# neuronika/neuronika

Hardware: NVIDIA H100
Metric: forward+backward GFLOP/s (higher is better)
Workload: dtype bf16

## Files before the change

neuronika_b200/csrc/nk_gemm_tc.cu:

```cuda
#include "nk_internal.cuh"
#include "nk_ptx.cuh"

namespace {

constexpr int BLOCK_M = 128;
constexpr int BLOCK_K = 64;
constexpr int WGMMA_K = 16;
constexpr int kNumThreads = 384;
constexpr uint32_t kSmemLimit = 232448;
constexpr int kEpiCols = 64;
constexpr uint32_t kEpiStageBytes = 2 * 64 * kEpiCols * 4;

struct GemmParams {
  int64_t M, N, K;
  int64_t ldc;
  void* C;
  const void* bias;
  float alpha, beta;
  int bias_bf16;
  int bias_per_row;
  int relu;
  const void* mask;
  float* colsum;
  int num_m_blocks, num_n_blocks, num_k_blocks;
  uint32_t a_lbo, a_sbo, a_kstep;
  uint32_t b_lbo, b_sbo, b_kstep;
  int rs_world, m_rot;
  int64_t rs_rows;
  void* rs_dst[8];
  int batch, a_batched, b_batched, batch_reduce, splits;
  int64_t c_batch_stride;
  int tma_store;
};

__device__ __forceinline__ int tile_m_block(const GemmParams& p, int tile) {
  const int t = tile % p.num_m_blocks;
  if (p.rs_world == 0) return t;
  const int owner = (t + p.m_rot) % p.rs_world;
  return owner * (p.num_m_blocks / p.rs_world) + t / p.rs_world;
}

constexpr int kGroupM = 16;
__device__ __forceinline__ void tile_coords(const GemmParams& p, int tile, int& m_blk, int& n_blk) {
  if (p.rs_world) {
    m_blk = tile_m_block(p, tile);
    n_blk = tile / p.num_m_blocks;
    return;
  }
  const int group_size = kGroupM * p.num_n_blocks;
  const int group = tile / group_size, in_group = tile - group * group_size;
  const int first_m = group * kGroupM;
  const int gm = min(p.num_m_blocks - first_m, kGroupM);
  m_blk = first_m + in_group % gm;
  n_blk = in_group / gm;
}

template <int BLOCK_N>
struct Cfg {
  static constexpr uint32_t A_BYTES = BLOCK_M * BLOCK_K * 2;
  static constexpr uint32_t B_BYTES = BLOCK_N * BLOCK_K * 2;
  static constexpr uint32_t STAGE_BYTES = A_BYTES + B_BYTES;
  static constexpr int kStagesMax = (kSmemLimit - 2048 - kEpiStageBytes) / STAGE_BYTES;
  static constexpr int kStages = kStagesMax > 8 ? 8 : kStagesMax;
  static constexpr uint32_t SMEM_BYTES = kStages * STAGE_BYTES + 2048 + kEpiStageBytes;
};

__device__ __forceinline__ void scale_and_bias(const GemmParams& p, int64_t row, int64_t col0, const uint32_t* r, bool full,
                                               float* v) {
#pragma unroll
  for (int j = 0; j < 32; ++j) v[j] = __fmul_rn(p.alpha, __uint_as_float(r[j]));
  if (p.bias && p.bias_per_row) {
    const float b = p.bias_bf16 ? __bfloat162float(static_cast<const __nv_bfloat16*>(p.bias)[row]) : static_cast<const float*>(p.bias)[row];
#pragma unroll
    for (int j = 0; j < 32; ++j) v[j] += b;
  } else if (p.bias) {
    if (full && (reinterpret_cast<uintptr_t>(p.bias) & 15) == 0) {
      if (p.bias_bf16) {
        const uint4* bp = reinterpret_cast<const uint4*>(static_cast<const __nv_bfloat16*>(p.bias) + col0);
#pragma unroll
        for (int q = 0; q < 4; ++q) {
          const uint4 w = __ldg(bp + q);
          const uint32_t ww[4] = {w.x, w.y, w.z, w.w};
#pragma unroll
          for (int i = 0; i < 4; ++i) {
            v[q * 8 + 2 * i] += __uint_as_float(ww[i] << 16);
            v[q * 8 + 2 * i + 1] += __uint_as_float(ww[i] & 0xffff0000u);
          }
        }
      } else {
        const float4* bp = reinterpret_cast<const float4*>(static_cast<const float*>(p.bias) + col0);
#pragma unroll
        for (int q = 0; q < 8; ++q) {
          const float4 w = __ldg(bp + q);
          v[q * 4] += w.x, v[q * 4 + 1] += w.y, v[q * 4 + 2] += w.z, v[q * 4 + 3] += w.w;
        }
      }
    } else {
#pragma unroll
      for (int j = 0; j < 32; ++j)
        if (col0 + j < p.N)
          v[j] += p.bias_bf16 ? __bfloat162float(static_cast<const __nv_bfloat16*>(p.bias)[col0 + j])
                              : static_cast<const float*>(p.bias)[col0 + j];
    }
  }
}

template <typename TC>
__device__ __forceinline__ void epilogue_colsum_chunk32(const GemmParams& p, int64_t row, int64_t col0, const uint32_t* r,
                                                        int lane, bool vec_ok) {
  float v[32];
  const bool live = row < p.M;
  const TC* mrow = (p.mask && live) ? static_cast<const TC*>(p.mask) + row * p.ldc + col0 : nullptr;
  const bool full = col0 + 32 <= p.N;
#pragma unroll
  for (int j = 0; j < 32; ++j) v[j] = (live && col0 + j < p.N) ? p.alpha * __uint_as_float(r[j]) : 0.f;
  if (mrow) {
    if (full && vec_ok) {
      constexpr int V = 16 / sizeof(TC);
#pragma unroll
      for (int q = 0; q < 32 / V; ++q) {
        NkVec<TC> mk;
        mk.load(mrow + q * V);
#pragma unroll
        for (int i = 0; i < V; ++i) v[q * V + i] = mk.get(i) > 0.f ? v[q * V + i] : 0.f;
      }
    } else {
#pragma unroll
      for (int j = 0; j < 32; ++j)
        if (col0 + j < p.N) v[j] = nk_to_f32<TC>(mrow[j]) > 0.f ? v[j] : 0.f;
    }
  }
#pragma unroll
  for (int j = 0; j < 32; ++j) v[j] = nk_to_f32<TC>(nk_from_f32<TC>(v[j]));
#pragma unroll
  for (int off = 16; off >= 1; off >>= 1) {
    const bool upper = (lane & off) != 0;
#pragma unroll
    for (int i = 0; i < off; ++i) {
      const float send = upper ? v[i] : v[i + off];
      const float keep = upper ? v[i + off] : v[i];
      v[i] = keep + __shfl_xor_sync(0xffffffffu, send, off);
    }
  }
  if (col0 + lane < p.N) atomicAdd(p.colsum + col0 + lane, v[0]);
}

template <typename TC>
__device__ __forceinline__ void epilogue_store_chunk32(const GemmParams& p, int64_t row, int64_t col0, const uint32_t* r,
                                                       int ncols, bool vec_ok, int64_t c_off = 0, bool atomic = false) {
  TC* crow = static_cast<TC*>(p.C) + c_off + row * p.ldc + col0;
  if (atomic) {
    if constexpr (sizeof(TC) == 4) {
#pragma unroll
      for (int j = 0; j < 32; ++j)
        if (j < ncols && col0 + j < p.N) atomicAdd(reinterpret_cast<float*>(crow) + j, p.alpha * __uint_as_float(r[j]));
    }
    return;
  }
  if (p.rs_world) {
    const int owner = int(row / p.rs_rows);
    crow = static_cast<TC*>(p.rs_dst[owner]) + (row - owner * p.rs_rows) * p.ldc + col0;
  }
  float v[32];
  const bool full = (col0 + 32 <= p.N) && ncols == 32;
  scale_and_bias(p, row, col0, r, full, v);
  const TC* mrow = p.mask ? static_cast<const TC*>(p.mask) + row * p.ldc + col0 : nullptr;
  if (full && vec_ok) {
    constexpr int V = 16 / sizeof(TC);
    if (mrow) {
#pragma unroll
      for (int q = 0; q < 32 / V; ++q) {
        NkVec<TC> mk;
        mk.load(mrow + q * V);
#pragma unroll
        for (int i = 0; i < V; ++i) v[q * V + i] = mk.get(i) > 0.f ? v[q * V + i] : 0.f;
      }
    }
    if (p.beta != 0.f) {
#pragma unroll
      for (int q = 0; q < 32 / V; ++q) {
        NkVec<TC> c;
        c.load(crow + q * V);
#pragma unroll
        for (int i = 0; i < V; ++i) v[q * V + i] += p.beta * c.get(i);
      }
    }
    if (p.relu) {
#pragma unroll
      for (int j = 0; j < 32; ++j) v[j] = v[j] > 0.f ? v[j] : 0.f;
    }
#pragma unroll
    for (int q = 0; q < 32 / V; ++q) {
      NkVec<TC> o;
#pragma unroll
      for (int i = 0; i < V; ++i) o.set(i, v[q * V + i]);
      o.store(crow + q * V);
    }
  } else {
#pragma unroll
    for (int j = 0; j < 32; ++j) {
      if (j < ncols && col0 + j < p.N) {
        float x = v[j];
        if (mrow) x = nk_to_f32<TC>(mrow[j]) > 0.f ? x : 0.f;
        if (p.beta != 0.f) x += p.beta * nk_to_f32<TC>(crow[j]);
        if (p.relu) x = x > 0.f ? x : 0.f;
        crow[j] = nk_from_f32<TC>(x);
      }
    }
  }
}

__device__ __forceinline__ int epi_index(int row, int col) {
  return row * kEpiCols + ((((col >> 2) ^ (row & 7))) << 2) + (col & 3);
}

__device__ __forceinline__ float col_bias(const GemmParams& p, int64_t col) {
  if (col >= p.N) return 0.f;
  return p.bias_bf16 ? __bfloat162float(static_cast<const __nv_bfloat16*>(p.bias)[col]) : static_cast<const float*>(p.bias)[col];
}

__device__ __forceinline__ float epi_value(const GemmParams& p, float acc, float bias) {
  float v = __fmul_rn(p.alpha, acc);
  if (p.bias) v += bias;
  return p.relu ? (v > 0.f ? v : 0.f) : v;
}

template <int BLOCK_N, bool A_MN, bool B_MN, typename TC, bool BATCH = false>
__global__ void __launch_bounds__(kNumThreads, 1)
gemm_tc_kernel(const __grid_constant__ CUtensorMap tmap_a, const __grid_constant__ CUtensorMap tmap_b,
               const __grid_constant__ CUtensorMap tmap_c, const GemmParams p) {
  using C_ = Cfg<BLOCK_N>;
  constexpr int kStages = C_::kStages;
  constexpr int kStoreCols = 128 / int(sizeof(TC));
  constexpr bool kTmaStore = !BATCH && BLOCK_N % kStoreCols == 0;
  static_assert(2 * 2 * 64 * 128 <= kEpiStageBytes, "staging buffers");
  extern __shared__ uint8_t smem_raw[];
  const uint32_t smem_base = (ptx::smem_u32(smem_raw) + 1023u) & ~1023u;
  const uint32_t smem_a0 = smem_base;
  const uint32_t smem_b0 = smem_base + kStages * C_::A_BYTES;
  const uint32_t bar_base = smem_base + kStages * C_::STAGE_BYTES;
  auto full_bar = [&](int s) { return bar_base + 8u * s; };
  auto empty_bar = [&](int s) { return bar_base + 8u * (kStages + s); };
  const uint32_t epi_stage = bar_base + 1024;
  float* epi = reinterpret_cast<float*>(smem_raw + (epi_stage - ptx::smem_u32(smem_raw)));

  const int wg = threadIdx.x >> 7;
  const int lane = threadIdx.x & 31;

  if (threadIdx.x == 0) {
    ptx::prefetch_tmap(&tmap_a);
    ptx::prefetch_tmap(&tmap_b);
    if (kTmaStore && p.tma_store) ptx::prefetch_tmap(&tmap_c);
    for (int s = 0; s < kStages; ++s) {
      ptx::mbar_init(full_bar(s), 1);
      ptx::mbar_init(empty_bar(s), 2);
    }
    ptx::fence_barrier_init();
  }
  __syncthreads();

  const int tiles_mn = p.num_m_blocks * p.num_n_blocks;
  const int num_tiles = BATCH ? tiles_mn * (p.batch_reduce ? p.splits : p.batch) : tiles_mn;
  auto batch_range = [&](int outer, int& b0, int& b1) {
    if (!p.batch_reduce) {
      b0 = outer, b1 = outer + 1;
    } else {
      const int per = (p.batch + p.splits - 1) / p.splits;
      b0 = outer * per;
      b1 = min(p.batch, b0 + per);
    }
  };

  if (wg == 0) {
    ptx::setmaxnreg_dec<40>();
    if (threadIdx.x == 0) {
      int stage = 0;
      uint32_t phase = 0;
      for (int tile = blockIdx.x; tile < num_tiles; tile += gridDim.x) {
        int m_blk, n_blk, b0 = 0, b1 = 1;
        tile_coords(p, BATCH ? tile % tiles_mn : tile, m_blk, n_blk);
        if (BATCH) batch_range(tile / tiles_mn, b0, b1);
        const int m0 = m_blk * BLOCK_M, n0 = n_blk * BLOCK_N;
        for (int bb = b0; bb < b1; ++bb)
        for (int kb = 0; kb < p.num_k_blocks; ++kb) {
          ptx::mbar_wait_spin(empty_bar(stage), phase ^ 1u);
          ptx::mbar_expect_tx(full_bar(stage), C_::STAGE_BYTES);
          const int k0 = kb * BLOCK_K;
          const uint32_t sa = smem_a0 + stage * C_::A_BYTES;
          const uint32_t sb = smem_b0 + stage * C_::B_BYTES;
          if (A_MN) {
#pragma unroll
            for (int c = 0; c < BLOCK_M / 64; ++c) {
              if (BATCH && p.a_batched)
                ptx::tma_load_3d(sa + c * (64 * BLOCK_K * 2), &tmap_a, full_bar(stage), m0 + c * 64, k0, bb);
              else
                ptx::tma_load_2d(sa + c * (64 * BLOCK_K * 2), &tmap_a, full_bar(stage), m0 + c * 64, k0);
            }
          } else {
            if (BATCH && p.a_batched)
              ptx::tma_load_3d(sa, &tmap_a, full_bar(stage), k0, m0, bb);
            else
              ptx::tma_load_2d(sa, &tmap_a, full_bar(stage), k0, m0);
          }
          if (B_MN) {
#pragma unroll
            for (int c = 0; c < BLOCK_N / 64; ++c) {
              if (BATCH && p.b_batched)
                ptx::tma_load_3d(sb + c * (64 * BLOCK_K * 2), &tmap_b, full_bar(stage), n0 + c * 64, k0, bb);
              else
                ptx::tma_load_2d(sb + c * (64 * BLOCK_K * 2), &tmap_b, full_bar(stage), n0 + c * 64, k0);
            }
          } else {
            if (BATCH && p.b_batched)
              ptx::tma_load_3d(sb, &tmap_b, full_bar(stage), k0, n0, bb);
            else
              ptx::tma_load_2d(sb, &tmap_b, full_bar(stage), k0, n0);
          }
          if (++stage == kStages) {
            stage = 0;
            phase ^= 1u;
          }
        }
      }
    }
    return;
  }

  ptx::setmaxnreg_inc<232>();
  const int cw = wg - 1;
  const int t = threadIdx.x & 127;
  const int warp = t >> 5;
  const bool vec_ok = ((p.ldc * int64_t(sizeof(TC))) % 16 == 0) && ((reinterpret_cast<uintptr_t>(p.C) & 15) == 0) &&
                      ((reinterpret_cast<uintptr_t>(p.mask) & 15) == 0);
  float* stg = epi + cw * (64 * kEpiCols);
  const uint32_t a_off = uint32_t(cw) * (64 * BLOCK_K * 2);
  float acc[BLOCK_N / 2];
  int stage = 0;
  uint32_t phase = 0;
  uint32_t store_buf = 0;
  for (int tile = blockIdx.x; tile < num_tiles; tile += gridDim.x) {
    int m_blk, n_blk;
    tile_coords(p, BATCH ? tile % tiles_mn : tile, m_blk, n_blk);
    int k_total = p.num_k_blocks;
    if (BATCH) {
      int b0, b1;
      batch_range(tile / tiles_mn, b0, b1);
      k_total *= (b1 - b0);
    }
    int prev_stage = 0;
    for (int kb = 0; kb < k_total; ++kb) {
      ptx::mbar_wait_spin(full_bar(stage), phase);
      const uint64_t adesc = ptx::make_smem_desc_sw128(smem_a0 + stage * C_::A_BYTES + a_off, p.a_lbo, p.a_sbo);
      const uint64_t bdesc = ptx::make_smem_desc_sw128(smem_b0 + stage * C_::B_BYTES, p.b_lbo, p.b_sbo);
      ptx::fence_regs(acc);
      ptx::wgmma_fence();
#pragma unroll
      for (int k = 0; k < BLOCK_K / WGMMA_K; ++k)
        ptx::Wgmma<BLOCK_N>::template mma<int(A_MN), int(B_MN)>(acc, adesc + uint64_t((k * p.a_kstep) >> 4),
                                                                 bdesc + uint64_t((k * p.b_kstep) >> 4), (kb | k) != 0 ? 1u : 0u);
      ptx::wgmma_commit();
      ptx::wgmma_wait<1>();
      ptx::fence_regs(acc);
      if (kb > 0 && t == 0) ptx::mbar_arrive(empty_bar(prev_stage));
      prev_stage = stage;
      if (++stage == kStages) {
        stage = 0;
        phase ^= 1u;
      }
    }
    ptx::wgmma_wait<0>();
    ptx::fence_regs(acc);
    if (t == 0) ptx::mbar_arrive(empty_bar(prev_stage));

    if constexpr (kTmaStore) {
      if (p.tma_store) {
        const int fr = warp * 16 + (lane >> 2);
        const int q = lane & 3;
        const int row0 = m_blk * BLOCK_M + cw * 64;
        const uint32_t stg0 = epi_stage + uint32_t(cw) * (2 * 64 * 128);
#pragma unroll
        for (int ch = 0; ch < BLOCK_N / kStoreCols; ++ch) {
          const uint32_t buf = stg0 + store_buf * (64 * 128);
          if (t == 0) ptx::tma_store_wait_read<1>();
          ptx::named_barrier(1 + cw, 128);
          const int64_t col0 = int64_t(n_blk) * BLOCK_N + ch * kStoreCols;
#pragma unroll
          for (int jj = 0; jj < kStoreCols / 8; ++jj) {
            const int j = (ch * (kStoreCols / 8) + jj) * 4;
            const int64_t col = col0 + jj * 8 + 2 * q;
            float b0 = 0.f, b1 = 0.f;
            if (p.bias) b0 = col_bias(p, col), b1 = col_bias(p, col + 1);
            const float v0 = epi_value(p, acc[j], b0), v1 = epi_value(p, acc[j + 1], b1);
            const float v2 = epi_value(p, acc[j + 2], b0), v3 = epi_value(p, acc[j + 3], b1);
            if constexpr (sizeof(TC) == 2) {
              const uint32_t off = fr * 128 + ((jj ^ (fr & 7)) << 4) + 4 * q;
              const __nv_bfloat162 lo = __floats2bfloat162_rn(v0, v1), hi = __floats2bfloat162_rn(v2, v3);
              ptx::st_shared_b32(buf + off, *reinterpret_cast<const uint32_t*>(&lo));
              ptx::st_shared_b32(buf + off + 8 * 128, *reinterpret_cast<const uint32_t*>(&hi));
            } else {
              const uint32_t off = fr * 128 + (((2 * jj + (q >> 1)) ^ (fr & 7)) << 4) + (q & 1) * 8;
              ptx::st_shared_v2_f32(buf + off, v0, v1);
              ptx::st_shared_v2_f32(buf + off + 8 * 128, v2, v3);
            }
          }
          ptx::fence_proxy_async();
          ptx::named_barrier(1 + cw, 128);
          if (t == 0) {
            if (row0 < p.M && col0 < p.N) ptx::tma_store_2d(&tmap_c, buf, int(col0), row0);
            ptx::tma_store_commit();
          }
          store_buf ^= 1u;
        }
        continue;
      }
    }

    const int64_t c_off = (BATCH && !p.batch_reduce) ? int64_t(tile / tiles_mn) * p.c_batch_stride : 0;
    const bool atomic = BATCH && p.batch_reduce;
    const int fr = warp * 16 + (lane >> 2);
    const int fc = (lane & 3) * 2;
    const int half = warp >> 1;
    const int rloc = (warp & 1) * 32 + lane;
    const int64_t row = int64_t(m_blk) * BLOCK_M + cw * 64 + rloc;
    constexpr int kChunks = (BLOCK_N + kEpiCols - 1) / kEpiCols;
#pragma unroll
    for (int ch = 0; ch < kChunks; ++ch) {
      constexpr int kFullBlocks = kEpiCols / 8;
      ptx::named_barrier(1 + cw, 128);
#pragma unroll
      for (int nb = 0; nb < kFullBlocks; ++nb) {
        if (ch * kFullBlocks + nb < BLOCK_N / 8) {
          const int j = (ch * kFullBlocks + nb) * 4;
          *reinterpret_cast<float2*>(stg + epi_index(fr, nb * 8 + fc)) = make_float2(acc[j], acc[j + 1]);
          *reinterpret_cast<float2*>(stg + epi_index(fr + 8, nb * 8 + fc)) = make_float2(acc[j + 2], acc[j + 3]);
        }
      }
      ptx::named_barrier(1 + cw, 128);
      const int chunk_cols = BLOCK_N - ch * kEpiCols < kEpiCols ? BLOCK_N - ch * kEpiCols : kEpiCols;
      if (!vec_ok && !p.colsum && !p.mask && !p.rs_world) {
        const int64_t col_base = int64_t(n_blk) * BLOCK_N + ch * kEpiCols;
        for (int rr = 0; rr < 16; ++rr) {
          const int srow = warp * 16 + rr;
          const int64_t grow = int64_t(m_blk) * BLOCK_M + cw * 64 + srow;
          if (grow >= p.M) break;
          float rb = 0.f;
          if (p.bias && p.bias_per_row)
            rb = p.bias_bf16 ? __bfloat162float(static_cast<const __nv_bfloat16*>(p.bias)[grow]) : static_cast<const float*>(p.bias)[grow];
          for (int c = lane; c < chunk_cols; c += 32) {
            const int64_t col = col_base + c;
            if (col >= p.N) break;
            float v = __fmul_rn(p.alpha, stg[epi_index(srow, c)]);
            TC* cp = static_cast<TC*>(p.C) + c_off + grow * p.ldc + col;
            if (atomic) {
              if constexpr (sizeof(TC) == 4) atomicAdd(reinterpret_cast<float*>(cp), v);
              continue;
            }
            if (p.bias) {
              v += p.bias_per_row ? rb
                                  : (p.bias_bf16 ? __bfloat162float(static_cast<const __nv_bfloat16*>(p.bias)[col])
                                                 : static_cast<const float*>(p.bias)[col]);
            }
            if (p.beta != 0.f) v += p.beta * nk_to_f32<TC>(*cp);
            if (p.relu) v = v > 0.f ? v : 0.f;
            *cp = nk_from_f32<TC>(v);
          }
        }
        continue;
      }
      const int ncols = min(32, chunk_cols - half * 32);
      if (ncols > 0) {
        uint32_t r[32];
#pragma unroll
        for (int q = 0; q < 8; ++q) {
          float4 v = make_float4(0.f, 0.f, 0.f, 0.f);
          if (q * 4 < ncols) v = *reinterpret_cast<const float4*>(stg + epi_index(rloc, half * 32 + q * 4));
          r[4 * q] = __float_as_uint(v.x), r[4 * q + 1] = __float_as_uint(v.y);
          r[4 * q + 2] = __float_as_uint(v.z), r[4 * q + 3] = __float_as_uint(v.w);
        }
        const int64_t col0 = int64_t(n_blk) * BLOCK_N + ch * kEpiCols + half * 32;
        if (p.colsum && col0 < p.N) epilogue_colsum_chunk32<TC>(p, row, col0, r, lane, vec_ok);
        if (row < p.M && col0 < p.N) epilogue_store_chunk32<TC>(p, row, col0, r, ncols, vec_ok, c_off, atomic);
      }
    }
  }
  if (kTmaStore && p.tma_store && t == 0) ptx::tma_store_wait<0>();
}

typedef CUresult (*EncodeTiledFn)(CUtensorMap*, CUtensorMapDataType, cuuint32_t, void*, const cuuint64_t*,
                                  const cuuint64_t*, const cuuint32_t*, const cuuint32_t*, CUtensorMapInterleave,
                                  CUtensorMapSwizzle, CUtensorMapL2promotion, CUtensorMapFloatOOBfill);

int make_tmap_2d(nk_ctx* ctx, CUtensorMap* tm, const void* base, int64_t rows, int64_t cols, int64_t ld,
                 uint32_t box_cols, uint32_t box_rows, int dtype = NK_BF16) {
  if (!ctx->encode_tiled) return nk_set_error(ctx, NK_ERR_CUDA, "cuTensorMapEncodeTiled unavailable");
  cuuint64_t dims[2] = {(cuuint64_t)cols, (cuuint64_t)rows};
// ... 68 lines not shown
}

}

bool nk_gemm_wgmma_supported(int transA, int transB, int64_t M, int64_t N, int64_t K, const void* A, int64_t lda,
                             const void* B, int64_t ldb) {
  (void)transA;
  (void)transB;
  if (M <= 0 || N <= 0 || K <= 0) return false;
  if ((reinterpret_cast<uintptr_t>(A) & 15) || (reinterpret_cast<uintptr_t>(B) & 15)) return false;
  if ((lda * 2) % 16 != 0 || (ldb * 2) % 16 != 0) return false;
  if (M > (int64_t(1) << 30) || N > (int64_t(1) << 30) || K > (int64_t(1) << 30)) return false;
  return true;
}

int nk_gemm_wgmma(nk_ctx* ctx, int transA, int transB, int64_t M, int64_t N, int64_t K, float alpha, const void* A,
                  int64_t lda, const void* B, int64_t ldb, float beta, void* C, int64_t ldc, int c_dtype,
                  const void* bias, int bias_dtype, int relu, const void* mask, float* colsum) {
  if (!nk_gemm_wgmma_supported(transA, transB, M, N, K, A, lda, B, ldb)) return NK_ERR_UNSUPPORTED;
  if (colsum && (N <= 16 || beta != 0.f)) return NK_ERR_UNSUPPORTED;
  const bool a_mn = transA != 0;
  const bool b_mn = transB == 0;
  int block_n = 256;
  if (N <= 16 && !b_mn)
    block_n = 16;
  else if (N <= 32 && !b_mn)
    block_n = 32;
  else if (N <= 64)
    block_n = 64;
  else if (N <= 128)
    block_n = 128;

  GemmParams p;
  p.M = M;
  p.N = N;
  p.K = K;
  p.ldc = ldc;
  p.C = C;
  p.bias = bias;
  p.alpha = alpha;
  p.beta = beta;
  p.bias_bf16 = bias_dtype == NK_BF16;
  p.bias_per_row = 0;
  p.relu = relu;
  p.mask = mask;
  p.colsum = colsum;
  p.batch = 1, p.a_batched = p.b_batched = p.batch_reduce = 0, p.splits = 1, p.c_batch_stride = 0;
  p.num_m_blocks = int((M + BLOCK_M - 1) / BLOCK_M);
  p.num_n_blocks = 0;
  p.num_k_blocks = int((K + BLOCK_K - 1) / BLOCK_K);
  p.rs_world = 0;
  p.m_rot = 0;
  p.rs_rows = M;
  for (int i = 0; i < 8; ++i) p.rs_dst[i] = nullptr;
  if (ctx->rs_world > 1) {
    if (M % (int64_t(ctx->rs_world) * BLOCK_M) != 0 || beta != 0.f || c_dtype != NK_F32)
      return nk_set_error(ctx, NK_ERR_INVALID_ARG, "wgmma gemm: reduce-scatter epilogue needs M %% (world*128) == 0, "
                          "beta == 0 and f32 output");
    p.rs_world = ctx->rs_world;
    p.rs_rows = M / ctx->rs_world;
    p.m_rot = ctx->rs_rank;
    for (int i = 0; i < ctx->rs_world; ++i) p.rs_dst[i] = ctx->rs_dst[i];
  }
  p.a_lbo = a_mn ? BLOCK_K * 128 : 16;
  p.a_sbo = 1024;
  p.a_kstep = a_mn ? WGMMA_K * 128 : WGMMA_K * 2;
  p.b_lbo = b_mn ? BLOCK_K * 128 : 16;
  p.b_sbo = 1024;
  p.b_kstep = b_mn ? WGMMA_K * 128 : WGMMA_K * 2;

  CUtensorMap ta, tb;
  int rc;
  if (a_mn)
    rc = make_tmap_2d(ctx, &ta, A, K, M, lda, 64, BLOCK_K);
  else
    rc = make_tmap_2d(ctx, &ta, A, M, K, lda, BLOCK_K, BLOCK_M);
  if (rc) return rc;
  if (b_mn)
    rc = make_tmap_2d(ctx, &tb, B, K, N, ldb, 64, BLOCK_K);
  else
    rc = make_tmap_2d(ctx, &tb, B, N, K, ldb, BLOCK_K, (uint32_t)block_n);
  if (rc) return rc;
  const int64_t c_size = int64_t(nk_dtype_size(c_dtype));
  CUtensorMap tc;
  memset(&tc, 0, sizeof(tc));
  p.tma_store = beta == 0.f && !mask && !colsum && !p.rs_world && (block_n * c_size) % 128 == 0 &&
                (reinterpret_cast<uintptr_t>(C) & 15) == 0 && (ldc * c_size) % 16 == 0 && (N * c_size) % 16 == 0;
  if (p.tma_store) {
    rc = make_tmap_2d(ctx, &tc, C, M, N, ldc, uint32_t(128 / c_size), 64, c_dtype);
    if (rc) return rc;
  }

  static const char* names[2][2][5] = {
      {{"wgmma_nt_128x256", "wgmma_nt_128x128", "wgmma_nt_128x64", "wgmma_nt_128x32", "wgmma_nt_128x16"},
       {"wgmma_nn_128x256", "wgmma_nn_128x128", "wgmma_nn_128x64", "", ""}},
      {{"wgmma_tt_128x256", "wgmma_tt_128x128", "wgmma_tt_128x64", "wgmma_tt_128x32", "wgmma_tt_128x16"},
       {"wgmma_tn_128x256", "wgmma_tn_128x128", "wgmma_tn_128x64", "", ""}}};
  const int bi = block_n == 256 ? 0 : block_n == 128 ? 1 : block_n == 64 ? 2 : block_n == 32 ? 3 : 4;
  ctx->last_gemm_kernel = names[a_mn][b_mn][bi];

#define NK_TC(AM, BM_)                                                              \
  (c_dtype == NK_BF16 ? launch_bn<AM, BM_, __nv_bfloat16>(ctx, block_n, ta, tb, tc, p) \
                      : launch_bn<AM, BM_, float>(ctx, block_n, ta, tb, tc, p))
  if (!a_mn && !b_mn) return NK_TC(false, false);
  if (!a_mn && b_mn) return NK_TC(false, true);
  if (a_mn && !b_mn) return NK_TC(true, false);
  return NK_TC(true, true);
#undef NK_TC
}

static int make_tmap_3d(nk_ctx* ctx, CUtensorMap* tm, const void* base, int64_t rows, int64_t cols, int64_t ld, int64_t batch,
                        int64_t batch_stride, uint32_t box_cols, uint32_t box_rows) {
  if (!ctx->encode_tiled) return nk_set_error(ctx, NK_ERR_CUDA, "cuTensorMapEncodeTiled unavailable");
  cuuint64_t dims[3] = {(cuuint64_t)cols, (cuuint64_t)rows, (cuuint64_t)batch};
  cuuint64_t strides[2] = {(cuuint64_t)ld * 2, (cuuint64_t)batch_stride * 2};
  cuuint32_t box[3] = {box_cols, box_rows, 1};
  cuuint32_t estr[3] = {1, 1, 1};
  CUresult r = reinterpret_cast<EncodeTiledFn>(ctx->encode_tiled)(
      tm, CU_TENSOR_MAP_DATA_TYPE_BFLOAT16, 3, const_cast<void*>(base), dims, strides, box, estr,
      CU_TENSOR_MAP_INTERLEAVE_NONE, CU_TENSOR_MAP_SWIZZLE_128B, CU_TENSOR_MAP_L2_PROMOTION_L2_256B,
      CU_TENSOR_MAP_FLOAT_OOB_FILL_NONE);
  if (r != CUDA_SUCCESS)
    return nk_set_error(ctx, NK_ERR_CUDA, "cuTensorMapEncodeTiled (3-d) failed (%d) rows=%lld cols=%lld ld=%lld batch=%lld stride=%lld",
                        (int)r, (long long)rows, (long long)cols, (long long)ld, (long long)batch, (long long)batch_stride);
  return NK_OK;
}

int nk_gemm_wgmma_batched(nk_ctx* ctx, int transA, int transB, int64_t M, int64_t N, int64_t K, float alpha, const void* A,
                            int64_t lda, int64_t strideA, const void* B, int64_t ldb, int64_t strideB, void* C, int64_t ldc,
                            int64_t strideC, int64_t batch, int c_dtype, const void* row_bias, int bias_dtype, int relu,
                            int reduce) {
  if (!nk_gemm_wgmma_supported(transA, transB, M, N, K, A, lda, B, ldb)) return NK_ERR_UNSUPPORTED;
  if (batch < 1 || batch > (int64_t(1) << 30) || (strideA * 2) % 16 != 0 || (strideB * 2) % 16 != 0) return NK_ERR_UNSUPPORTED;
  if (reduce && c_dtype != NK_F32) return NK_ERR_UNSUPPORTED;
  const bool a_mn = transA != 0, b_mn = transB == 0;
  int block_n = N <= 64 ? 64 : (N <= 128 ? 128 : 256);
  GemmParams p;
  p.M = M, p.N = N, p.K = K, p.ldc = ldc, p.C = C;
  p.bias = row_bias, p.bias_bf16 = bias_dtype == NK_BF16, p.bias_per_row = 1;
  p.alpha = alpha, p.beta = 0.f, p.relu = relu, p.mask = nullptr, p.colsum = nullptr;
  p.num_m_blocks = int((M + BLOCK_M - 1) / BLOCK_M);
  p.num_n_blocks = 0;
  p.num_k_blocks = int((K + BLOCK_K - 1) / BLOCK_K);
  p.rs_world = 0, p.m_rot = 0, p.rs_rows = M;
  for (int i = 0; i < 8; ++i) p.rs_dst[i] = nullptr;
  p.batch = int(batch), p.a_batched = strideA != 0, p.b_batched = strideB != 0, p.batch_reduce = reduce ? 1 : 0, p.splits = 1;
  p.c_batch_stride = strideC;
  p.tma_store = 0;
  p.a_lbo = a_mn ? BLOCK_K * 128 : 16, p.a_sbo = 1024, p.a_kstep = a_mn ? WGMMA_K * 128 : WGMMA_K * 2;
  p.b_lbo = b_mn ? BLOCK_K * 128 : 16, p.b_sbo = 1024, p.b_kstep = b_mn ? WGMMA_K * 128 : WGMMA_K * 2;
  CUtensorMap ta, tb;
  int rc;
  if (p.a_batched)
    rc = a_mn ? make_tmap_3d(ctx, &ta, A, K, M, lda, batch, strideA, 64, BLOCK_K)
              : make_tmap_3d(ctx, &ta, A, M, K, lda, batch, strideA, BLOCK_K, BLOCK_M);
  else
    rc = a_mn ? make_tmap_2d(ctx, &ta, A, K, M, lda, 64, BLOCK_K) : make_tmap_2d(ctx, &ta, A, M, K, lda, BLOCK_K, BLOCK_M);
  if (rc) return rc;
  if (p.b_batched)
    rc = b_mn ? make_tmap_3d(ctx, &tb, B, K, N, ldb, batch, strideB, 64, BLOCK_K)
              : make_tmap_3d(ctx, &tb, B, N, K, ldb, batch, strideB, BLOCK_K, (uint32_t)block_n);
  else
    rc = b_mn ? make_tmap_2d(ctx, &tb, B, K, N, ldb, 64, BLOCK_K) : make_tmap_2d(ctx, &tb, B, N, K, ldb, BLOCK_K, (uint32_t)block_n);
  if (rc) return rc;
  CUtensorMap tc;
  memset(&tc, 0, sizeof(tc));
  ctx->last_gemm_kernel = "wgmma_batched";
#define NK_TCB(BN, AM, BM_)                                                                          \
  (c_dtype == NK_BF16 ? launch_cfg<BN, AM, BM_, __nv_bfloat16, true>(ctx, ta, tb, tc, p)              \
                      : launch_cfg<BN, AM, BM_, float, true>(ctx, ta, tb, tc, p))
// ... 89 lines not shown
```

neuronika_b200/csrc/nk_ptx.cuh:

```cuda
#pragma once
#include <cuda.h>
#include <stdint.h>

namespace ptx {

__device__ __forceinline__ uint32_t smem_u32(const void* p) {
  return static_cast<uint32_t>(__cvta_generic_to_shared(p));
}

__device__ __forceinline__ bool elect_one() {
  uint32_t pred = 0;
  asm volatile(
      "{\n\t"
      ".reg .b32 %%rx;\n\t"
      ".reg .pred %%px;\n\t"
      "elect.sync %%rx|%%px, %1;\n\t"
      "@%%px mov.s32 %0, 1;\n\t"
      "}\n"
      : "+r"(pred)
      : "r"(0xFFFFFFFFu));
  return pred != 0;
}

__device__ __forceinline__ void mbar_init(uint32_t bar, uint32_t count) {
// ... 7 lines not shown
}
__device__ __forceinline__ void mbar_expect_tx(uint32_t bar, uint32_t bytes) {
  asm volatile("mbarrier.arrive.expect_tx.shared::cta.b64 _, [%0], %1;" ::"r"(bar), "r"(bytes) : "memory");
}
__device__ __forceinline__ void mbar_arrive(uint32_t bar) {
  asm volatile("mbarrier.arrive.shared::cta.b64 _, [%0];" ::"r"(bar) : "memory");
}
__device__ __forceinline__ bool mbar_try_wait(uint32_t bar, uint32_t parity) {
  uint32_t ok;
  asm volatile(
      "{\n\t"
      ".reg .pred p;\n\t"
      "mbarrier.try_wait.parity.shared::cta.b64 p, [%1], %2;\n\t"
      "selp.u32 %0, 1, 0, p;\n\t"
      "}\n"
      : "=r"(ok)
      : "r"(bar), "r"(parity)
      : "memory");
  return ok != 0;
}
__device__ __forceinline__ bool mbar_try_wait_sleep(uint32_t bar, uint32_t parity) {
  uint32_t ok;
  asm volatile(
      "{\n\t"
      ".reg .pred p;\n\t"
      "mbarrier.try_wait.parity.shared::cta.b64 p, [%1], %2, %3;\n\t"
      "selp.u32 %0, 1, 0, p;\n\t"
      "}\n"
      : "=r"(ok)
      : "r"(bar), "r"(parity), "r"(0x989680u)
      : "memory");
  return ok != 0;
}
__device__ __forceinline__ void mbar_wait_spin(uint32_t bar, uint32_t parity) {
  while (!mbar_try_wait_sleep(bar, parity)) {
  }
}

__device__ __forceinline__ void mbar_wait_relaxed(uint32_t bar, uint32_t parity) {
  if (mbar_try_wait(bar, parity)) return;
  uint32_t spins = 0, ns = 32;
  long long t0 = 0;
  while (!mbar_try_wait_sleep(bar, parity)) {
    __nanosleep(ns);
    if (ns < 512) ns <<= 1;
    if ((++spins & 63u) != 0) continue;
    const long long now = clock64();
    if (t0 == 0) t0 = now;
    if (now - t0 > (1ll << 32)) {
      printf("nk_b200: mbarrier watchdog: block %d thread %d bar 0x%x parity %u\n", blockIdx.x, threadIdx.x, bar,
             parity);
      __trap();
    }
  }
}

__device__ __forceinline__ void prefetch_tmap(const CUtensorMap* tmap) {
  asm volatile("prefetch.tensormap [%0];" ::"l"(reinterpret_cast<uint64_t>(tmap)) : "memory");
}
__device__ __forceinline__ void tma_load_2d(uint32_t smem_dst, const CUtensorMap* tmap, uint32_t bar, int32_t c0,
                                            int32_t c1) {
  asm volatile(
      "cp.async.bulk.tensor.2d.shared::cluster.global.mbarrier::complete_tx::bytes [%0], [%1, {%3, %4}], [%2];" ::"r"(
          smem_dst),
      "l"(reinterpret_cast<uint64_t>(tmap)), "r"(bar), "r"(c0), "r"(c1)
      : "memory");
}
__device__ __forceinline__ void tma_load_3d(uint32_t smem_dst, const CUtensorMap* tmap, uint32_t bar, int32_t c0,
                                            int32_t c1, int32_t c2) {
  asm volatile(
      "cp.async.bulk.tensor.3d.shared::cluster.global.mbarrier::complete_tx::bytes [%0], [%1, {%3, %4, %5}], [%2];" ::
          "r"(smem_dst),
      "l"(reinterpret_cast<uint64_t>(tmap)), "r"(bar), "r"(c0), "r"(c1), "r"(c2)
      : "memory");
}
__device__ __forceinline__ void tma_load_4d(uint32_t smem_dst, const CUtensorMap* tmap, uint32_t bar, int32_t c0,
                                            int32_t c1, int32_t c2, int32_t c3) {
  asm volatile(
      "cp.async.bulk.tensor.4d.shared::cluster.global.mbarrier::complete_tx::bytes [%0], [%1, {%3, %4, %5, %6}], "
      "[%2];" ::"r"(smem_dst),
      "l"(reinterpret_cast<uint64_t>(tmap)), "r"(bar), "r"(c0), "r"(c1), "r"(c2), "r"(c3)
      : "memory");
}
__device__ __forceinline__ void tma_store_2d(const CUtensorMap* tmap, uint32_t smem_src, int32_t c0, int32_t c1) {
  asm volatile("cp.async.bulk.tensor.2d.global.shared::cta.bulk_group [%0, {%2, %3}], [%1];" ::"l"(
                   reinterpret_cast<uint64_t>(tmap)),
               "r"(smem_src), "r"(c0), "r"(c1)
               : "memory");
}
__device__ __forceinline__ void tma_store_4d(const CUtensorMap* tmap, uint32_t smem_src, int32_t c0, int32_t c1,
                                             int32_t c2, int32_t c3) {
  asm volatile("cp.async.bulk.tensor.4d.global.shared::cta.bulk_group [%0, {%2, %3, %4, %5}], [%1];" ::"l"(
                   reinterpret_cast<uint64_t>(tmap)),
               "r"(smem_src), "r"(c0), "r"(c1), "r"(c2), "r"(c3)
               : "memory");
}
__device__ __forceinline__ void tma_store_commit() { asm volatile("cp.async.bulk.commit_group;" ::: "memory"); }
__device__ __forceinline__ void st_shared_b32(uint32_t addr, uint32_t v) {
  asm volatile("st.shared.b32 [%0], %1;" ::"r"(addr), "r"(v) : "memory");
}
__device__ __forceinline__ void st_shared_v2_f32(uint32_t addr, float x, float y) {
  asm volatile("st.shared.v2.f32 [%0], {%1, %2};" ::"r"(addr), "f"(x), "f"(y) : "memory");
}
template <int N>
__device__ __forceinline__ void tma_store_wait_read() {
  asm volatile("cp.async.bulk.wait_group.read %0;" ::"n"(N) : "memory");
}
template <int N>
__device__ __forceinline__ void tma_store_wait() {
  asm volatile("cp.async.bulk.wait_group %0;" ::"n"(N) : "memory");
}


template <uint32_t R>
__device__ __forceinline__ void setmaxnreg_dec() { asm volatile("setmaxnreg.dec.sync.aligned.u32 %0;" ::"n"(R)); }
template <uint32_t R>
__device__ __forceinline__ void setmaxnreg_inc() { asm volatile("setmaxnreg.inc.sync.aligned.u32 %0;" ::"n"(R)); }
__device__ __forceinline__ void named_barrier(uint32_t id, uint32_t count) {
  asm volatile("bar.sync %0, %1;" ::"r"(id), "r"(count) : "memory");
}

__device__ __forceinline__ void wgmma_fence() { asm volatile("wgmma.fence.sync.aligned;" ::: "memory"); }
__device__ __forceinline__ void wgmma_commit() { asm volatile("wgmma.commit_group.sync.aligned;" ::: "memory"); }
template <int N>
__device__ __forceinline__ void wgmma_wait() {
  asm volatile("wgmma.wait_group.sync.aligned %0;" ::"n"(N) : "memory");
}
template <int R>
__device__ __forceinline__ void fence_regs(float (&d)[R]) {
#pragma unroll
  for (int i = 0; i < R; ++i) asm volatile("" : "+f"(d[i])::"memory");
}

__device__ __forceinline__ uint64_t make_smem_desc_sw128(uint32_t smem_addr, uint32_t lbo_bytes, uint32_t sbo_bytes) {
  uint64_t d = 0;
  d |= uint64_t((smem_addr >> 4) & 0x3FFFu);
  d |= uint64_t((lbo_bytes >> 4) & 0x3FFFu) << 16;
  d |= uint64_t((sbo_bytes >> 4) & 0x3FFFu) << 32;
  d |= uint64_t(1) << 62;
  return d;
}

template <int N>
struct Wgmma;
template <>
struct Wgmma<16> {
  template <int TA, int TB>
  __device__ __forceinline__ static void mma(float (&d)[8], uint64_t da, uint64_t db, uint32_t scale_d) {
    asm volatile(
        "{\n\t.reg .pred p;\n\tsetp.ne.b32 p, %10, 0;\n\t"
        "wgmma.mma_async.sync.aligned.m64n16k16.f32.bf16.bf16 "
        "{"
        "%0, %1, %2, %3, %4, %5, %6, %7"
        "}, %8, %9, p, 1, 1, %11, %12;\n\t}\n"
        : "+f"(d[0]), "+f"(d[1]), "+f"(d[2]), "+f"(d[3]), "+f"(d[4]), "+f"(d[5]), "+f"(d[6]), "+f"(d[7])
        : "l"(da), "l"(db), "r"(scale_d), "n"(TA), "n"(TB));
  }
};
template <>
struct Wgmma<32> {
  template <int TA, int TB>
  __device__ __forceinline__ static void mma(float (&d)[16], uint64_t da, uint64_t db, uint32_t scale_d) {
    asm volatile(
        "{\n\t.reg .pred p;\n\tsetp.ne.b32 p, %18, 0;\n\t"
        "wgmma.mma_async.sync.aligned.m64n32k16.f32.bf16.bf16 "
        "{"
        "%0, %1, %2, %3, %4, %5, %6, %7, %8, %9, %10, %11, %12, %13, %14, %15"
        "}, %16, %17, p, 1, 1, %19, %20;\n\t}\n"
        : "+f"(d[0]), "+f"(d[1]), "+f"(d[2]), "+f"(d[3]), "+f"(d[4]), "+f"(d[5]), "+f"(d[6]), "+f"(d[7]),
          "+f"(d[8]), "+f"(d[9]), "+f"(d[10]), "+f"(d[11]), "+f"(d[12]), "+f"(d[13]), "+f"(d[14]), "+f"(d[15])
        : "l"(da), "l"(db), "r"(scale_d), "n"(TA), "n"(TB));
  }
};
template <>
struct Wgmma<64> {
  template <int TA, int TB>
  __device__ __forceinline__ static void mma(float (&d)[32], uint64_t da, uint64_t db, uint32_t scale_d) {
    asm volatile(
        "{\n\t.reg .pred p;\n\tsetp.ne.b32 p, %34, 0;\n\t"
        "wgmma.mma_async.sync.aligned.m64n64k16.f32.bf16.bf16 "
        "{"
        "%0, %1, %2, %3, %4, %5, %6, %7, %8, %9, %10, %11, %12, %13, %14, %15, "
        "%16, %17, %18, %19, %20, %21, %22, %23, %24, %25, %26, %27, %28, %29, %30, %31"
        "}, %32, %33, p, 1, 1, %35, %36;\n\t}\n"
        : "+f"(d[0]), "+f"(d[1]), "+f"(d[2]), "+f"(d[3]), "+f"(d[4]), "+f"(d[5]), "+f"(d[6]), "+f"(d[7]),
// ... 69 lines not shown
```

Before: 742,700.

## Prefetch bias via bulk copy into shared memory and store epilogue with stmatrix

The producer warp now bulk-loads the tile's bias slice into shared memory, synchronised by a new full/empty mbarrier pair, so consumers no longer read bias from global memory per element. The bf16 epilogue writes the staging buffer with stmatrix.x4 instead of scalar 32-bit shared stores. Extra shared memory is reserved for the bias buffer and barriers, which may cut one pipeline stage for some tile sizes. The TMA-store path is now also gated on bias alignment.

```diff
diff --git a/neuronika_b200/csrc/nk_gemm_tc.cu b/neuronika_b200/csrc/nk_gemm_tc.cu
--- a/neuronika_b200/csrc/nk_gemm_tc.cu
+++ b/neuronika_b200/csrc/nk_gemm_tc.cu
@@ -60,9 +60,9 @@
   static constexpr uint32_t A_BYTES = BLOCK_M * BLOCK_K * 2;
   static constexpr uint32_t B_BYTES = BLOCK_N * BLOCK_K * 2;
   static constexpr uint32_t STAGE_BYTES = A_BYTES + B_BYTES;
-  static constexpr int kStagesMax = (kSmemLimit - 2048 - kEpiStageBytes) / STAGE_BYTES;
+  static constexpr int kStagesMax = (kSmemLimit - 3072 - kEpiStageBytes) / STAGE_BYTES;
   static constexpr int kStages = kStagesMax > 8 ? 8 : kStagesMax;
-  static constexpr uint32_t SMEM_BYTES = kStages * STAGE_BYTES + 2048 + kEpiStageBytes;
+  static constexpr uint32_t SMEM_BYTES = kStages * STAGE_BYTES + 3072 + kEpiStageBytes;
 };
 
 __device__ __forceinline__ void scale_and_bias(const GemmParams& p, int64_t row, int64_t col0, const uint32_t* r, bool full,
@@ -212,11 +212,6 @@
 
 __device__ __forceinline__ int epi_index(int row, int col) {
   return row * kEpiCols + ((((col >> 2) ^ (row & 7))) << 2) + (col & 3);
-}
-
-__device__ __forceinline__ float col_bias(const GemmParams& p, int64_t col) {
-  if (col >= p.N) return 0.f;
-  return p.bias_bf16 ? __bfloat162float(static_cast<const __nv_bfloat16*>(p.bias)[col]) : static_cast<const float*>(p.bias)[col];
 }
 
 __device__ __forceinline__ float epi_value(const GemmParams& p, float acc, float bias) {
@@ -241,8 +236,12 @@
   const uint32_t bar_base = smem_base + kStages * C_::STAGE_BYTES;
   auto full_bar = [&](int s) { return bar_base + 8u * s; };
   auto empty_bar = [&](int s) { return bar_base + 8u * (kStages + s); };
-  const uint32_t epi_stage = bar_base + 1024;
+  const uint32_t bias_full = bar_base + 8u * (2 * kStages);
+  const uint32_t bias_empty = bias_full + 8u;
+  const uint32_t bias_smem = bar_base + 1024;
+  const uint32_t epi_stage = bar_base + 2048;
   float* epi = reinterpret_cast<float*>(smem_raw + (epi_stage - ptx::smem_u32(smem_raw)));
+  const bool bias_copy = kTmaStore && p.tma_store && p.bias;
 
   const int wg = threadIdx.x >> 7;
   const int lane = threadIdx.x & 31;
@@ -255,6 +254,8 @@
       ptx::mbar_init(full_bar(s), 1);
       ptx::mbar_init(empty_bar(s), 2);
     }
+    ptx::mbar_init(bias_full, 1);
+    ptx::mbar_init(bias_empty, 2);
     ptx::fence_barrier_init();
   }
   __syncthreads();
@@ -315,6 +316,13 @@
               ptx::tma_load_3d(sb, &tmap_b, full_bar(stage), k0, n0, bb);
             else
               ptx::tma_load_2d(sb, &tmap_b, full_bar(stage), k0, n0);
+          }
+          if (bias_copy && kb == min(kStages, p.num_k_blocks) - 1) {
+            ptx::mbar_wait_spin(bias_empty, (((tile - blockIdx.x) / gridDim.x) & 1) ^ 1u);
+            const int esize = p.bias_bf16 ? 2 : 4;
+            const uint32_t bytes = uint32_t(min(int64_t(BLOCK_N), p.N - n0)) * esize;
+            ptx::mbar_expect_tx(bias_full, bytes);
+            ptx::bulk_load(bias_smem, static_cast<const uint8_t*>(p.bias) + int64_t(n0) * esize, bytes, bias_full);
           }
           if (++stage == kStages) {
             stage = 0;
@@ -378,29 +386,58 @@
         const int q = lane & 3;
         const int row0 = m_blk * BLOCK_M + cw * 64;
         const uint32_t stg0 = epi_stage + uint32_t(cw) * (2 * 64 * 128);
+        if (bias_copy) ptx::mbar_wait_spin(bias_full, ((tile - blockIdx.x) / gridDim.x) & 1);
+        const uint8_t* sbias = smem_raw + (bias_smem - ptx::smem_u32(smem_raw));
 #pragma unroll
         for (int ch = 0; ch < BLOCK_N / kStoreCols; ++ch) {
           const uint32_t buf = stg0 + store_buf * (64 * 128);
           if (t == 0) ptx::tma_store_wait_read<1>();
           ptx::named_barrier(1 + cw, 128);
           const int64_t col0 = int64_t(n_blk) * BLOCK_N + ch * kStoreCols;
+          float bias_c[kStoreCols / 4];
 #pragma unroll
           for (int jj = 0; jj < kStoreCols / 8; ++jj) {
-            const int j = (ch * (kStoreCols / 8) + jj) * 4;
-            const int64_t col = col0 + jj * 8 + 2 * q;
+            const int c = ch * kStoreCols + 8 * jj + 2 * q;
             float b0 = 0.f, b1 = 0.f;
-            if (p.bias) b0 = col_bias(p, col), b1 = col_bias(p, col + 1);
-            const float v0 = epi_value(p, acc[j], b0), v1 = epi_value(p, acc[j + 1], b1);
-            const float v2 = epi_value(p, acc[j + 2], b0), v3 = epi_value(p, acc[j + 3], b1);
-            if constexpr (sizeof(TC) == 2) {
-              const uint32_t off = fr * 128 + ((jj ^ (fr & 7)) << 4) + 4 * q;
-              const __nv_bfloat162 lo = __floats2bfloat162_rn(v0, v1), hi = __floats2bfloat162_rn(v2, v3);
-              ptx::st_shared_b32(buf + off, *reinterpret_cast<const uint32_t*>(&lo));
-              ptx::st_shared_b32(buf + off + 8 * 128, *reinterpret_cast<const uint32_t*>(&hi));
-            } else {
+            if (bias_copy) {
+              if (p.bias_bf16) {
+                const uint32_t w = *reinterpret_cast<const uint32_t*>(sbias + 2 * c);
+                b0 = __uint_as_float(w << 16), b1 = __uint_as_float(w & 0xffff0000u);
+              } else {
+                const float2 w = *reinterpret_cast<const float2*>(sbias + 4 * c);
+                b0 = w.x, b1 = w.y;
+              }
+              const int64_t col = col0 + 8 * jj + 2 * q;
+              if (col >= p.N) b0 = 0.f;
+              if (col + 1 >= p.N) b1 = 0.f;
+            }
+            bias_c[2 * jj] = b0, bias_c[2 * jj + 1] = b1;
+          }
+          if constexpr (sizeof(TC) == 2) {
+            const int srow = warp * 16 + ((lane >> 3) & 1) * 8 + (lane & 7);
+#pragma unroll
+            for (int jp = 0; jp < kStoreCols / 16; ++jp) {
+              uint32_t r[4];
+#pragma unroll
+              for (int h = 0; h < 2; ++h) {
+                const int jj = 2 * jp + h;
+                const int j = (ch * (kStoreCols / 8) + jj) * 4;
+                const float b0 = bias_c[2 * jj], b1 = bias_c[2 * jj + 1];
+                const __nv_bfloat162 lo = __floats2bfloat162_rn(epi_value(p, acc[j], b0), epi_value(p, acc[j + 1], b1));
+                const __nv_bfloat162 hi = __floats2bfloat162_rn(epi_value(p, acc[j + 2], b0), epi_value(p, acc[j + 3], b1));
+                r[2 * h] = *reinterpret_cast<const uint32_t*>(&lo);
+                r[2 * h + 1] = *reinterpret_cast<const uint32_t*>(&hi);
+              }
+              ptx::stmatrix_x4(buf + srow * 128 + (((2 * jp + (lane >> 4)) ^ (lane & 7)) << 4), r[0], r[1], r[2], r[3]);
+            }
+          } else {
+#pragma unroll
+            for (int jj = 0; jj < kStoreCols / 8; ++jj) {
+              const int j = (ch * (kStoreCols / 8) + jj) * 4;
+              const float b0 = bias_c[2 * jj], b1 = bias_c[2 * jj + 1];
               const uint32_t off = fr * 128 + (((2 * jj + (q >> 1)) ^ (fr & 7)) << 4) + (q & 1) * 8;
-              ptx::st_shared_v2_f32(buf + off, v0, v1);
-              ptx::st_shared_v2_f32(buf + off + 8 * 128, v2, v3);
+              ptx::st_shared_v2_f32(buf + off, epi_value(p, acc[j], b0), epi_value(p, acc[j + 1], b1));
+              ptx::st_shared_v2_f32(buf + off + 8 * 128, epi_value(p, acc[j + 2], b0), epi_value(p, acc[j + 3], b1));
             }
           }
           ptx::fence_proxy_async();
@@ -411,6 +448,7 @@
           }
           store_buf ^= 1u;
         }
+        if (bias_copy && t == 0) ptx::mbar_arrive(bias_empty);
         continue;
       }
     }
@@ -645,10 +683,12 @@
     rc = make_tmap_2d(ctx, &tb, B, N, K, ldb, BLOCK_K, (uint32_t)block_n);
   if (rc) return rc;
   const int64_t c_size = int64_t(nk_dtype_size(c_dtype));
+  const int64_t bias_size = bias ? int64_t(nk_dtype_size(bias_dtype)) : 0;
   CUtensorMap tc;
   memset(&tc, 0, sizeof(tc));
   p.tma_store = beta == 0.f && !mask && !colsum && !p.rs_world && (block_n * c_size) % 128 == 0 &&
-                (reinterpret_cast<uintptr_t>(C) & 15) == 0 && (ldc * c_size) % 16 == 0 && (N * c_size) % 16 == 0;
+                (reinterpret_cast<uintptr_t>(C) & 15) == 0 && (ldc * c_size) % 16 == 0 && (N * c_size) % 16 == 0 &&
+                (reinterpret_cast<uintptr_t>(bias) & 15) == 0 && (N * bias_size) % 16 == 0;
   if (p.tma_store) {
     rc = make_tmap_2d(ctx, &tc, C, M, N, ldc, uint32_t(128 / c_size), 64, c_dtype);
     if (rc) return rc;
diff --git a/neuronika_b200/csrc/nk_ptx.cuh b/neuronika_b200/csrc/nk_ptx.cuh
--- a/neuronika_b200/csrc/nk_ptx.cuh
+++ b/neuronika_b200/csrc/nk_ptx.cuh
@@ -113,6 +113,11 @@
       "l"(reinterpret_cast<uint64_t>(tmap)), "r"(bar), "r"(c0), "r"(c1), "r"(c2), "r"(c3)
       : "memory");
 }
+__device__ __forceinline__ void bulk_load(uint32_t smem_dst, const void* src, uint32_t bytes, uint32_t bar) {
+  asm volatile("cp.async.bulk.shared::cluster.global.mbarrier::complete_tx::bytes [%0], [%1], %2, [%3];" ::"r"(smem_dst),
+               "l"(reinterpret_cast<uint64_t>(src)), "r"(bytes), "r"(bar)
+               : "memory");
+}
 __device__ __forceinline__ void tma_store_2d(const CUtensorMap* tmap, uint32_t smem_src, int32_t c0, int32_t c1) {
   asm volatile("cp.async.bulk.tensor.2d.global.shared::cta.bulk_group [%0, {%2, %3}], [%1];" ::"l"(
                    reinterpret_cast<uint64_t>(tmap)),
@@ -127,11 +132,13 @@
                : "memory");
 }
 __device__ __forceinline__ void tma_store_commit() { asm volatile("cp.async.bulk.commit_group;" ::: "memory"); }
-__device__ __forceinline__ void st_shared_b32(uint32_t addr, uint32_t v) {
-  asm volatile("st.shared.b32 [%0], %1;" ::"r"(addr), "r"(v) : "memory");
-}
 __device__ __forceinline__ void st_shared_v2_f32(uint32_t addr, float x, float y) {
   asm volatile("st.shared.v2.f32 [%0], {%1, %2};" ::"r"(addr), "f"(x), "f"(y) : "memory");
+}
+__device__ __forceinline__ void stmatrix_x4(uint32_t addr, uint32_t r0, uint32_t r1, uint32_t r2, uint32_t r3) {
+  asm volatile("stmatrix.sync.aligned.m8n8.x4.shared.b16 [%0], {%1, %2, %3, %4};" ::"r"(addr), "r"(r0), "r"(r1), "r"(r2),
+               "r"(r3)
+               : "memory");
 }
 template <int N>
 __device__ __forceinline__ void tma_store_wait_read() {
```

After: 761,600 (median of 6 runs). 1.03x the previous value.
